# yewsiang/Transferable3D

Measured on AMD Instinct MI355X. Metric: frustums/sec fwd+bwd, higher is better.
Workload: dtype f32

## Files before the change

transferable3d_amd/csrc/bn_optim.hip:

```cpp
#include "common.h"
#include "poolbwd_dev.h"
#include "bn_dev.h"

namespace {

template <int GR, int CH = FC_CH>
__global__ __launch_bounds__(GR * CH) void k_bn_fwd_finalize(const t3d_bn_fwd_finalize_args p) {
  __shared__ double red[GR][CH];
  __shared__ float s_scsh[2 * CH];
  bn_fwd_finalize_body<GR, CH>(p, red, s_scsh, blockIdx.x);
}

__global__ __launch_bounds__(256) void k_pool_finalize(const t3d_pool_finalize_args p) {
  const int i = blockIdx.x * blockDim.x + threadIdx.x;
  if (i >= p.B * p.N) return;
  const int b = i / p.N, c = i % p.N;
  pool_pick_impl(p.pmax, p.pmin, p.pamax, p.pamin, p.tiles_per_frustum, p.N, b, c, p.scale[c], p.shift[c], p.pooled, p.ld_pooled,
                 p.argidx, p.ysel);
}

template <int GR, int CH = FC_CH>
__global__ __launch_bounds__(GR * CH) void k_bn_bwd_finalize(const t3d_bn_bwd_finalize_args p) {
  __shared__ double red[GR][CH];
  bn_bwd_finalize_body<GR, CH>(p, red, blockIdx.x, threadIdx.x);
}

__global__ __launch_bounds__(256) void k_dy_colsum(const t3d_dy_colsum_args p) { dy_colsum_body(p, blockIdx.x, threadIdx.x); }

__global__ __launch_bounds__(256) void k_reduce_slabs(const float* __restrict__ slab_base, float* __restrict__ grad_base,
                                                      const t3d_slab_desc* __restrict__ table) {
  __shared__ float4 part[8][32];
  reduce_slabs_body(slab_base, grad_base, table, part, blockIdx.x, blockIdx.y, gridDim.x);
}

__global__ __launch_bounds__(256) void k_pool_bwd_mid(const float* __restrict__ slab_base, float* __restrict__ grad_base,
                                                      const t3d_slab_desc* __restrict__ table, const int gx, const int n_reduce,
                                                      const t3d_pool_sparse_rows_args sp) {
  extern __shared__ __attribute__((aligned(16))) float smem[];
  const int b = blockIdx.x;
  if (b < n_reduce) {
    reduce_slabs_body(slab_base, grad_base, table, reinterpret_cast<float4(*)[32]>(smem), b % gx, b / gx, gx);
  } else {
    const int r = b - n_reduce, tiles = sp.B * sp.rows_per_frustum / 128;
    pool_sparse_rows_body(sp, smem, r % tiles, r / tiles);
  }
}

__global__ __launch_bounds__(64) void k_schedule_step(float* hyper, const t3d_schedule s) {
  if (blockIdx.x != 0) return;
  schedule_step_body(hyper, s, threadIdx.x);
}

__global__ __launch_bounds__(256) void k_adam_tf(float* __restrict__ w, const float* __restrict__ g, float* __restrict__ m,
                                                 float* __restrict__ v, int64_t n, const float* __restrict__ hyper,
                                                 float b1, float b2, float eps, float gscale) {
  const float lr_t = hyper[3];
  for (int64_t i = (int64_t)blockIdx.x * blockDim.x + threadIdx.x; i < n; i += (int64_t)gridDim.x * blockDim.x) {
    float mi = m[i], vi = v[i];
    const float dw = adam_tf_elem(g[i], mi, vi, lr_t, b1, b2, eps, gscale);
    m[i] = mi;
    v[i] = vi;
    w[i] -= dw;
  }
}

constexpr int ADAM_RANGE_ELEMS = 1024;
__global__ __launch_bounds__(256) void k_reduce_slabs_adam(const float* __restrict__ slab_base, float* __restrict__ grad_base,
                                                           const t3d_slab_desc* __restrict__ table, const int gx, const int n_reduce,
                                                           const t3d_adam_range* __restrict__ ranges, const int n_ranges,
                                                           const adam_tail ad) {
  __shared__ float4 part[8][32];
  const int b = blockIdx.x;
  if (b < n_reduce) {
    reduce_slabs_body<true>(slab_base, grad_base, table, part, b % gx, b / gx, gx, &ad);
    return;
  }
  const int r = b - n_reduce;
  int lo = 0, hi = n_ranges - 1;
  while (lo < hi) {
    const int mid = (lo + hi + 1) >> 1;
    if (ranges[mid].blk0 <= r) lo = mid; else hi = mid - 1;
  }
  const t3d_adam_range rg = ranges[lo];
  const float lr_t = ad.hyper[3];
  const int64_t i0 = (int64_t)(r - rg.blk0) * ADAM_RANGE_ELEMS + threadIdx.x;
#pragma unroll
  for (int u = 0; u < ADAM_RANGE_ELEMS / 256; ++u) {
    const int64_t i = i0 + 256 * u;
    if (i < rg.n) {
      const int64_t o = rg.off + i;
      float mi = ad.m[o], vi = ad.v[o];
      const float dw = adam_tf_elem(grad_base[o], mi, vi, lr_t, ad.b1, ad.b2, ad.eps, ad.gscale);
      ad.m[o] = mi;
      ad.v[o] = vi;
      ad.w[o] -= dw;
    }
  }
}

__global__ __launch_bounds__(256) void k_momentum_tf(float* __restrict__ w, const float* __restrict__ g, float* __restrict__ acc,
                                                     int64_t n, const float* __restrict__ hyper, float momentum, float gscale) {
  const float lr = hyper[1];
  for (int64_t i = (int64_t)blockIdx.x * blockDim.x + threadIdx.x; i < n; i += (int64_t)gridDim.x * blockDim.x) {
    const float a = fmaf(momentum, acc[i], g[i] * gscale);
    acc[i] = a;
    w[i] -= lr * a;
  }
}

__device__ __forceinline__ uint32_t mix_u32(uint64_t x) {
  x ^= x >> 33; x *= 0xff51afd7ed558ccdULL;
  x ^= x >> 33; x *= 0xc4ceb9fe1a85ec53ULL;
  x ^= x >> 33;
  return (uint32_t)(x >> 16);
}
__global__ __launch_bounds__(256) void k_dropout_mask(float* __restrict__ mask, int64_t n, float keep, uint32_t seed,
                                                      const float* __restrict__ hyper) {
  const uint64_t step = (uint64_t)hyper[0];
  const uint64_t key = ((uint64_t)seed << 32) ^ (step * 0x9E3779B97F4A7C15ULL);
  for (int64_t i = (int64_t)blockIdx.x * blockDim.x + threadIdx.x; i < n; i += (int64_t)gridDim.x * blockDim.x) {
    const uint32_t r = mix_u32(key + (uint64_t)i * 0xD6E8FEB86659FD93ULL);
    const float u = (float)(r >> 8) * (1.0f / 16777216.0f);
    mask[i] = u < keep ? 1.f : 0.f;
  }
}

}

extern "C" int t3d_abi_version(void) { return T3D_ABI_VERSION; }

static int fin_big_tiles() {
  static const int v = []() { const char* e = getenv("T3D_FIN_BIG"); const int x = e ? atoi(e) : 512; return x > 0 ? x : (1 << 30); }();
  return v;
}

static int fin_wide_tiles() {
  static const int v = []() { const char* e = getenv("T3D_FIN_WIDE"); const int x = e ? atoi(e) : 1024; return x > 0 ? x : (1 << 30); }();
  return v;
}

extern "C" int t3d_bn_fwd_finalize(const t3d_bn_fwd_finalize_args* a, t3d_stream_t stream) {
  if (!a || !a->gamma || !a->beta || !a->moving_mean || !a->moving_var || !a->scale || !a->shift || !a->mean ||
      !a->invstd)
    return T3D_ERR_ARG;
  if (a->is_training && (!a->psum || !a->psumsq || !a->decay || a->count <= 0)) return T3D_ERR_ARG;
  if (a->is_training && a->n_tiles >= fin_wide_tiles() && a->N <= FC_WIDE_MAX_N)
    T3D_LAUNCH((k_bn_fwd_finalize<FC_GR_WIDE, FC_CH_WIDE>), dim3((a->N + FC_CH_WIDE - 1) / FC_CH_WIDE), dim3(FC_GR_WIDE * FC_CH_WIDE), 0,
               static_cast<hipStream_t>(stream), *a);
  else if (a->is_training && a->n_tiles > fin_big_tiles())
    T3D_LAUNCH(k_bn_fwd_finalize<FC_GR_BIG>, dim3((a->N + FC_CH - 1) / FC_CH), dim3(FC_GR_BIG * FC_CH), 0, static_cast<hipStream_t>(stream), *a);
  else
    T3D_LAUNCH(k_bn_fwd_finalize<FC_GR>, dim3((a->N + FC_CH - 1) / FC_CH), dim3(FC_GR * FC_CH), 0, static_cast<hipStream_t>(stream), *a);
  T3D_CHECK_LAUNCH();
  return T3D_OK;
}

extern "C" int t3d_pool_finalize(const t3d_pool_finalize_args* a, t3d_stream_t stream) {
  if (!a || !a->scale || !a->shift || !a->pmax || !a->pmin || !a->pamax || !a->pamin || !a->pooled || !a->argidx ||
      !a->ysel)
    return T3D_ERR_ARG;
  T3D_LAUNCH(k_pool_finalize, dim3((a->B * a->N + 255) / 256), dim3(256), 0, static_cast<hipStream_t>(stream),
                     *a);
  T3D_CHECK_LAUNCH();
  return T3D_OK;
}

extern "C" int t3d_bn_bwd_finalize(const t3d_bn_bwd_finalize_args* a, t3d_stream_t stream) {
  const int rc = check_bn_bwd_finalize(a);
  if (rc != T3D_OK) return rc;
  if (a->psum_dz != nullptr && a->n_tiles >= fin_wide_tiles() && a->N <= FC_WIDE_MAX_N)
    T3D_LAUNCH((k_bn_bwd_finalize<FC_GR_WIDE, FC_CH_WIDE>), dim3((a->N + FC_CH_WIDE - 1) / FC_CH_WIDE), dim3(FC_GR_WIDE * FC_CH_WIDE), 0,
               static_cast<hipStream_t>(stream), *a);
  else if (a->psum_dz != nullptr && a->n_tiles > fin_big_tiles())
    T3D_LAUNCH(k_bn_bwd_finalize<FC_GR_BIG>, dim3((a->N + FC_CH - 1) / FC_CH), dim3(FC_GR_BIG * FC_CH), 0, static_cast<hipStream_t>(stream), *a);
  else
    T3D_LAUNCH(k_bn_bwd_finalize<FC_GR>, dim3((a->N + FC_CH - 1) / FC_CH), dim3(FC_GR * FC_CH), 0, static_cast<hipStream_t>(stream), *a);
  T3D_CHECK_LAUNCH();
  return T3D_OK;
}

extern "C" int t3d_dy_colsum(const t3d_dy_colsum_args* a, t3d_stream_t stream) {
  const int rc = check_dy_colsum(a);
  if (rc != T3D_OK) return rc;
  T3D_LAUNCH(k_dy_colsum, dim3((a->B * a->N + 255) / 256), dim3(256), 0, static_cast<hipStream_t>(stream), *a);
  T3D_CHECK_LAUNCH();
  return T3D_OK;
}

extern "C" int t3d_reduce_slabs(const float* slab_base, float* grad_base, const t3d_slab_desc* table_dev, int n_tensors,
                                int max_numel, t3d_stream_t stream) {
  if (!slab_base || !grad_base || !table_dev || n_tensors <= 0) return T3D_ERR_ARG;
  int gx = (max_numel / 4 + 31) / 32;
  if (gx > 256) gx = 256;
  if (gx < 1) gx = 1;
  T3D_LAUNCH(k_reduce_slabs, dim3(gx, n_tensors), dim3(256), 0, static_cast<hipStream_t>(stream), slab_base,
                     grad_base, table_dev);
  T3D_CHECK_LAUNCH();
  return T3D_OK;
}

extern "C" int t3d_schedule_step(float* hyper, const t3d_schedule* s, t3d_stream_t stream) {
  if (!hyper || !s) return T3D_ERR_ARG;
  T3D_LAUNCH(k_schedule_step, dim3(1), dim3(64), 0, static_cast<hipStream_t>(stream), hyper, *s);
  T3D_CHECK_LAUNCH();
  return T3D_OK;
}

extern "C" int t3d_adam_tf_step(float* params, const float* grads, float* m, float* v, int64_t n, const float* hyper,
                                float beta1, float beta2, float eps, float grad_scale, t3d_stream_t stream) {
  if (!params || !grads || !m || !v || !hyper || n <= 0) return T3D_ERR_ARG;
  int64_t blocks = (n + 255) / 256;
  if (blocks > 2048) blocks = 2048;
  T3D_LAUNCH(k_adam_tf, dim3((unsigned)blocks), dim3(256), 0, static_cast<hipStream_t>(stream), params, grads, m,
                     v, n, hyper, beta1, beta2, eps, grad_scale);
  T3D_CHECK_LAUNCH();
  return T3D_OK;
}

extern "C" int t3d_reduce_slabs_adam(const float* slab_base, float* grad_base, const t3d_slab_desc* table_dev, int n_tensors,
                                     int max_numel, float* params, float* m, float* v, const t3d_adam_range* ranges_dev, int n_ranges,
                                     int n_range_blocks, const float* hyper, float beta1, float beta2, float eps, float grad_scale,
                                     t3d_stream_t stream) {
  if (!slab_base || !grad_base || !table_dev || n_tensors <= 0 || !params || !m || !v || !hyper) return T3D_ERR_ARG;
  if (n_ranges < 0 || n_range_blocks < 0 || (n_ranges == 0) != (n_range_blocks == 0) || (n_ranges > 0 && !ranges_dev)) return T3D_ERR_ARG;
  int gx = (max_numel / 4 + 31) / 32;
  if (gx > 256) gx = 256;
  if (gx < 1) gx = 1;
  const int n_reduce = gx * n_tensors;
  const adam_tail ad = {params, m, v, hyper, beta1, beta2, eps, grad_scale};
  T3D_LAUNCH(k_reduce_slabs_adam, dim3(n_reduce + n_range_blocks), dim3(256), 0, static_cast<hipStream_t>(stream), slab_base, grad_base,
             table_dev, gx, n_reduce, ranges_dev, n_ranges, ad);
  T3D_CHECK_LAUNCH();
  return T3D_OK;
}

extern "C" int t3d_momentum_step(float* params, const float* grads, float* accum, int64_t n, const float* hyper, float momentum,
                                 float grad_scale, t3d_stream_t stream) {
  if (!params || !grads || !accum || !hyper || n <= 0) return T3D_ERR_ARG;
  int64_t blocks = (n + 255) / 256;
  if (blocks > 2048) blocks = 2048;
  T3D_LAUNCH(k_momentum_tf, dim3((unsigned)blocks), dim3(256), 0, static_cast<hipStream_t>(stream), params, grads, accum, n, hyper,
             momentum, grad_scale);
  T3D_CHECK_LAUNCH();
  return T3D_OK;
}

__global__ __launch_bounds__(256) void k_cast_bf16(const float* __restrict__ src, bf16_t* __restrict__ dst, int64_t n) {
  const int64_t stride = (int64_t)gridDim.x * 256 * 8;
  for (int64_t i = ((int64_t)blockIdx.x * 256 + threadIdx.x) * 8; i < n; i += stride) {
    if (i + 8 <= n) {
      const float4 a = *reinterpret_cast<const float4*>(src + i), b = *reinterpret_cast<const float4*>(src + i + 4);
      const bf16x8 h = {(bf16_t)a.x, (bf16_t)a.y, (bf16_t)a.z, (bf16_t)a.w, (bf16_t)b.x, (bf16_t)b.y, (bf16_t)b.z, (bf16_t)b.w};
      *reinterpret_cast<bf16x8*>(dst + i) = h;
    } else {
      for (int64_t j = i; j < n; ++j) dst[j] = (bf16_t)src[j];
    }
  }
}

extern "C" int t3d_cast_bf16(const float* src, void* dst, int64_t n, t3d_stream_t stream) {
  if (!src || !dst || n <= 0 || (reinterpret_cast<uintptr_t>(src) & 15) || (reinterpret_cast<uintptr_t>(dst) & 15)) return T3D_ERR_ARG;
  int64_t blocks = (n + 2047) / 2048;
  if (blocks > 2048) blocks = 2048;
  T3D_LAUNCH(k_cast_bf16, dim3((unsigned)blocks), dim3(256), 0, static_cast<hipStream_t>(stream), src, static_cast<bf16_t*>(dst), n);
  T3D_CHECK_LAUNCH();
  return T3D_OK;
}

extern "C" int t3d_dropout_mask(float* mask, int64_t n, float keep_prob, uint32_t seed, const float* hyper,
                                t3d_stream_t stream) {
  if (!mask || !hyper || n <= 0) return T3D_ERR_ARG;
  int64_t blocks = (n + 255) / 256;
  if (blocks > 4096) blocks = 4096;
  T3D_LAUNCH(k_dropout_mask, dim3((unsigned)blocks), dim3(256), 0, static_cast<hipStream_t>(stream), mask, n,
                     keep_prob, seed, hyper);
  T3D_CHECK_LAUNCH();
  return T3D_OK;
}

extern "C" int t3d_pool_bwd_mid(const float* slab_base, float* grad_base, const t3d_slab_desc* table_dev, int n_tensors,
                                int max_numel, const t3d_pool_sparse_rows_args* a, t3d_stream_t stream) {
  if (!slab_base || !grad_base || !table_dev || n_tensors <= 0) return T3D_ERR_ARG;
  const int rc = check_sparse_rows(a);
  if (rc != T3D_OK) return rc;
  int gx = (max_numel / 4 + 31) / 32;
  if (gx > 256) gx = 256;
  if (gx < 1) gx = 1;
  const int n_reduce = gx * n_tensors;
  const long M = (long)a->B * a->rows_per_frustum;
  const int n_sparse = (int)(M / 128) * (a->K / SR_KC);
  const size_t lds = sparse_rows_lds(a->N);
  static size_t allowed = 0;
  if (lds > 64 * 1024 && lds > allowed) {
    (void)hipFuncSetAttribute(reinterpret_cast<const void*>(k_pool_bwd_mid), hipFuncAttributeMaxDynamicSharedMemorySize, (int)lds);
    allowed = lds;
  }
  T3D_LAUNCH(k_pool_bwd_mid, dim3(n_reduce + n_sparse), dim3(256), lds, static_cast<hipStream_t>(stream), slab_base, grad_base,
             table_dev, gx, n_reduce, *a);
  T3D_CHECK_LAUNCH();
  return T3D_OK;
}
```

transferable3d_amd/csrc/poolbwd.hip:

```cpp
#include "poolbwd_dev.h"

namespace {

__global__ __launch_bounds__(256) void k_pool_bwd_prep(const t3d_pool_bwd_prep_args p) {
  extern __shared__ __attribute__((aligned(16))) float smem[];
  pool_bwd_prep_body(p, smem, blockIdx.x, blockIdx.y, blockIdx.z);
}
__global__ __launch_bounds__(256) void k_pool_sparse_rows(const t3d_pool_sparse_rows_args p) {
  extern __shared__ __attribute__((aligned(16))) float smem[];
  pool_sparse_rows_body(p, smem, blockIdx.x, blockIdx.y);
}
template <class XT>
__global__ __launch_bounds__(256) void k_act_colsum(const t3d_act_colsum_args p) {
  extern __shared__ __attribute__((aligned(16))) float smem[];
  act_colsum_body<XT>(p, smem, blockIdx.x);
}
template <class XT>
__global__ __launch_bounds__(256) void k_pool_wgrad_finish(const t3d_pool_wgrad_finish_args p) {
  extern __shared__ __attribute__((aligned(16))) float smem[];
  pool_wgrad_finish_body<XT>(p, smem, blockIdx.x, blockIdx.y);
}

}

extern "C" int t3d_pool_bwd_prep(const t3d_pool_bwd_prep_args* a, t3d_stream_t stream) {
  const int rc = check_prep(a);
  if (rc != T3D_OK) return rc;
  T3D_LAUNCH(k_pool_bwd_prep, dim3(a->K / 32, a->K / 32, (a->N + PCH - 1) / PCH), dim3(256), PREP_LDS,
             static_cast<hipStream_t>(stream), *a);
  T3D_CHECK_LAUNCH();
  return T3D_OK;
}

extern "C" int t3d_pool_sparse_rows(const t3d_pool_sparse_rows_args* a, t3d_stream_t stream) {
  const int rc = check_sparse_rows(a);
  if (rc != T3D_OK) return rc;
  const size_t lds = sparse_rows_lds(a->N);
  static size_t allowed = 0;
  if (lds > 64 * 1024 && lds > allowed) {
    (void)hipFuncSetAttribute(reinterpret_cast<const void*>(k_pool_sparse_rows), hipFuncAttributeMaxDynamicSharedMemorySize,
                              (int)lds);
    allowed = lds;
  }
  const long M = (long)a->B * a->rows_per_frustum;
  T3D_LAUNCH(k_pool_sparse_rows, dim3(M / 128, a->K / SR_KC), dim3(256), lds, static_cast<hipStream_t>(stream), *a);
  T3D_CHECK_LAUNCH();
  return T3D_OK;
}

extern "C" int t3d_act_colsum(const t3d_act_colsum_args* a, t3d_stream_t stream) {
  const int rc = check_colsum(a);
  if (rc != T3D_OK) return rc;
  if (a->a.dtype == T3D_BF16) T3D_LAUNCH(k_act_colsum<bf16_t>, dim3(a->M / 128), dim3(256), COLSUM_LDS, static_cast<hipStream_t>(stream), *a);
  else T3D_LAUNCH(k_act_colsum<float>, dim3(a->M / 128), dim3(256), COLSUM_LDS, static_cast<hipStream_t>(stream), *a);
  T3D_CHECK_LAUNCH();
  return T3D_OK;
}

extern "C" int t3d_pool_wgrad_finish(const t3d_pool_wgrad_finish_args* a, t3d_stream_t stream) {
  const int rc = check_finish(a);
  if (rc != T3D_OK) return rc;
  const size_t lds = finish_lds(a->K);
  if (a->a.dtype == T3D_BF16) T3D_LAUNCH(k_pool_wgrad_finish<bf16_t>, dim3(a->K / FK, a->N / FN), dim3(256), lds, static_cast<hipStream_t>(stream), *a);
  else T3D_LAUNCH(k_pool_wgrad_finish<float>, dim3(a->K / FK, a->N / FN), dim3(256), lds, static_cast<hipStream_t>(stream), *a);
  T3D_CHECK_LAUNCH();
  return T3D_OK;
}
```

Baseline: 28140.

## Add per-wave register-accumulating sparse-rows kernel with counting-sort row bucketing

Adds a new sparse-rows backward path in which each wave gathers the argmax hits for its row subset, counting-sorts them by row in LDS, then streams weight rows with batched, software-pipelined float2 loads and accumulates each output row in registers. It replaces the tiled shared-memory accumulation kernel whenever the per-wave LDS fits in 64KB, both standalone and inside the fused pool_bwd_mid launch, where sparse blocks are now ordered before the reduce blocks. The aim is to avoid touching a large LDS tile per block, at the cost of serial per-wave sorting and inline-asm stores. An environment variable can force the old tiled path.

```diff
diff --git a/transferable3d_amd/csrc/bn_optim.hip b/transferable3d_amd/csrc/bn_optim.hip
--- a/transferable3d_amd/csrc/bn_optim.hip
+++ b/transferable3d_amd/csrc/bn_optim.hip
@@ -1,5 +1,6 @@
 #include "common.h"
 #include "poolbwd_dev.h"
+#include "sparse_rows_dev.h"
 #include "bn_dev.h"
 
 namespace {
@@ -43,6 +44,20 @@
   } else {
     const int r = b - n_reduce, tiles = sp.B * sp.rows_per_frustum / 128;
     pool_sparse_rows_body(sp, smem, r % tiles, r / tiles);
+  }
+}
+
+__global__ __launch_bounds__(256) void k_pool_bwd_mid_reg(const float* __restrict__ slab_base, float* __restrict__ grad_base,
+                                                          const t3d_slab_desc* __restrict__ table, const int gx, const int n_sparse,
+                                                          const t3d_pool_sparse_rows_args sp) {
+  extern __shared__ __attribute__((aligned(16))) float smem[];
+  const int b = blockIdx.x;
+  if (b < n_sparse) {
+    const int tiles = sp.B * sp.rows_per_frustum / 128;
+    pool_sparse_rows_reg_body(sp, reinterpret_cast<int*>(smem), b % tiles, b / tiles);
+  } else {
+    const int r = b - n_sparse;
+    reduce_slabs_body(slab_base, grad_base, table, reinterpret_cast<float4(*)[32]>(smem), r % gx, r / gx, gx);
   }
 }
 
@@ -289,6 +304,13 @@
   const int n_reduce = gx * n_tensors;
   const long M = (long)a->B * a->rows_per_frustum;
   const int n_sparse = (int)(M / 128) * (a->K / SR_KC);
+  if (!sparse_rows_take_tile(a->N)) {
+    const size_t rlds = sparse_rows_reg_lds(a->N) > 8 * 32 * sizeof(float4) ? sparse_rows_reg_lds(a->N) : 8 * 32 * sizeof(float4);
+    T3D_LAUNCH(k_pool_bwd_mid_reg, dim3(n_reduce + n_sparse), dim3(256), rlds, static_cast<hipStream_t>(stream), slab_base, grad_base,
+               table_dev, gx, n_sparse, *a);
+    T3D_CHECK_LAUNCH();
+    return T3D_OK;
+  }
   const size_t lds = sparse_rows_lds(a->N);
   static size_t allowed = 0;
   if (lds > 64 * 1024 && lds > allowed) {
diff --git a/transferable3d_amd/csrc/poolbwd.hip b/transferable3d_amd/csrc/poolbwd.hip
--- a/transferable3d_amd/csrc/poolbwd.hip
+++ b/transferable3d_amd/csrc/poolbwd.hip
@@ -1,4 +1,5 @@
 #include "poolbwd_dev.h"
+#include "sparse_rows_dev.h"
 
 namespace {
 
@@ -9,6 +10,10 @@
 __global__ __launch_bounds__(256) void k_pool_sparse_rows(const t3d_pool_sparse_rows_args p) {
   extern __shared__ __attribute__((aligned(16))) float smem[];
   pool_sparse_rows_body(p, smem, blockIdx.x, blockIdx.y);
+}
+__global__ __launch_bounds__(256) void k_pool_sparse_rows_reg(const t3d_pool_sparse_rows_args p) {
+  extern __shared__ __attribute__((aligned(16))) int smem_i[];
+  pool_sparse_rows_reg_body(p, smem_i, blockIdx.x, blockIdx.y);
 }
 template <class XT>
 __global__ __launch_bounds__(256) void k_act_colsum(const t3d_act_colsum_args p) {
@@ -35,6 +40,12 @@
 extern "C" int t3d_pool_sparse_rows(const t3d_pool_sparse_rows_args* a, t3d_stream_t stream) {
   const int rc = check_sparse_rows(a);
   if (rc != T3D_OK) return rc;
+  const long M = (long)a->B * a->rows_per_frustum;
+  if (!sparse_rows_take_tile(a->N)) {
+    T3D_LAUNCH(k_pool_sparse_rows_reg, dim3(M / 128, a->K / SR_KC), dim3(256), sparse_rows_reg_lds(a->N), static_cast<hipStream_t>(stream), *a);
+    T3D_CHECK_LAUNCH();
+    return T3D_OK;
+  }
   const size_t lds = sparse_rows_lds(a->N);
   static size_t allowed = 0;
   if (lds > 64 * 1024 && lds > allowed) {
@@ -42,7 +53,6 @@
                               (int)lds);
     allowed = lds;
   }
-  const long M = (long)a->B * a->rows_per_frustum;
   T3D_LAUNCH(k_pool_sparse_rows, dim3(M / 128, a->K / SR_KC), dim3(256), lds, static_cast<hipStream_t>(stream), *a);
   T3D_CHECK_LAUNCH();
   return T3D_OK;
diff --git a/transferable3d_amd/csrc/sparse_rows_dev.h b/transferable3d_amd/csrc/sparse_rows_dev.h
--- /dev/null
+++ b/transferable3d_amd/csrc/sparse_rows_dev.h
@@ -0,0 +1,227 @@
+#pragma once
+#include <cstdlib>
+#include <cstring>
+#include "poolbwd_dev.h"
+
+namespace {
+
+#ifndef SRR_BATCH_N
+#define SRR_BATCH_N 16
+#endif
+constexpr int SRR_BATCH = SRR_BATCH_N;
+
+#ifdef T3D_TRACE_SPARSE
+#define SRR_CLOCK(slot) srr_clk[slot] = (int)wall_clock64()
+#else
+#define SRR_CLOCK(slot) do {} while (0)
+#endif
+typedef float srr_f2 __attribute__((ext_vector_type(2)));
+constexpr size_t SRR_MAX_LDS = 64 * 1024;
+
+inline size_t sparse_rows_reg_lds(int N) { return (size_t)4 * (2 * (size_t)N + 64) * sizeof(int); }
+
+inline bool sparse_rows_take_tile(int N) {
+  const char* e = getenv("T3D_SPARSE_ROWS");
+  return (e != nullptr && strcmp(e, "tile") == 0) || sparse_rows_reg_lds(N) > SRR_MAX_LDS;
+}
+
+__device__ __forceinline__ void srr_wave_sync() {
+  __builtin_amdgcn_fence(__ATOMIC_RELEASE, "wavefront");
+  __builtin_amdgcn_wave_barrier();
+  __builtin_amdgcn_fence(__ATOMIC_ACQUIRE, "wavefront");
+}
+
+__device__ __forceinline__ unsigned long long srr_peers(int key, bool ok) {
+  unsigned long long m = __ballot(ok);
+#pragma unroll
+  for (int k = 0; k < 5; ++k) {
+    const bool bit = (key >> k) & 1;
+    const unsigned long long bk = __ballot(bit);
+    m &= bit ? bk : ~bk;
+  }
+  return m;
+}
+
+__device__ __forceinline__ void pool_sparse_rows_reg_body(const t3d_pool_sparse_rows_args& p, int* smem, int bx, int by) {
+  const int tid = threadIdx.x, lane = tid & 63, w = tid >> 6;
+  int* raw = smem + (size_t)w * (2 * p.N + 64);
+  int* srt = raw + p.N;
+  int* cur = srt + p.N;
+  const int row0 = bx * 128, kc0 = by * SR_KC;
+  const int b = row0 / p.rows_per_frustum, rin0 = row0 - b * p.rows_per_frustum;
+  const unsigned long long lt = (1ull << lane) - 1ull;
+  const bool gated = p.row_live != nullptr;
+
+#ifdef T3D_TRACE_SPARSE
+  int srr_clk[4];
+#endif
+  SRR_CLOCK(0);
+  cur[lane] = 0;
+  int cnt = 0;
+  for (int nb = 0; nb < p.N; nb += 64 * SR_PRE) {
+    int rr[SR_PRE];
+#pragma unroll
+    for (int q = 0; q < SR_PRE; ++q) {
+      const int n = nb + 64 * q + lane;
+      rr[q] = p.argidx[(size_t)b * p.N + min(n, p.N - 1)];
+    }
+#pragma unroll
+    for (int q = 0; q < SR_PRE; ++q) {
+      if (nb + 64 * q < p.N) {
+        const int n = nb + 64 * q + lane;
+        const int r = rr[q] - rin0;
+        const bool hit = n < p.N && r >= 0 && r < 128 && (r & 3) == w;
+        const unsigned long long m = __ballot(hit);
+        if (hit) raw[cnt + __popcll(m & lt)] = n | (r << 16);
+        cnt += __popcll(m);
+      }
+    }
+  }
+  cnt = __builtin_amdgcn_readfirstlane(cnt);
+  srr_wave_sync();
+  SRR_CLOCK(1);
+
+  for (int c0 = 0; c0 < cnt; c0 += 64) {
+    const bool ok = c0 + lane < cnt;
+    const int rl = raw[min(c0 + lane, cnt - 1)] >> 18;
+    const unsigned long long peers = srr_peers(rl, ok);
+    int base = 0;
+    if (ok) base = cur[rl];
+    srr_wave_sync();
+    if (ok) cur[rl] = base + __popcll(peers);
+    srr_wave_sync();
+  }
+  const int mycnt = lane < 32 ? cur[lane] : 0;
+  int incl = mycnt;
+#pragma unroll
+  for (int d = 1; d < 32; d *= 2) {
+    const int t = __shfl_up(incl, d, 64);
+    if (lane >= d) incl += t;
+  }
+  srr_wave_sync();
+  if (lane < 32) cur[lane] = incl - mycnt;
+  srr_wave_sync();
+  for (int c0 = 0; c0 < cnt; c0 += 64) {
+    const bool ok = c0 + lane < cnt;
+    const int e = raw[min(c0 + lane, cnt - 1)];
+    const int rl = e >> 18;
+    const unsigned long long peers = srr_peers(rl, ok);
+    int base = 0;
+    if (ok) {
+      base = cur[rl];
+      srt[base + __popcll(peers & lt)] = e;
+    }
+    srr_wave_sync();
+    if (ok) cur[rl] = base + __popcll(peers);
+    srr_wave_sync();
+  }
+
+  SRR_CLOCK(2);
+
+  if (cnt > 0) {
+    const int elast = __builtin_amdgcn_readfirstlane(raw[cnt - 1]);
+    const int rlast = (cnt % SR_UNROLL) != 0 ? elast >> 16 : -1;
+    const float2 wlast = *reinterpret_cast<const float2*>(p.wc + (size_t)(elast & 0xffff) * p.K + kc0 + 2 * lane);
+    srr_f2 acc = {0.f, 0.f};
+    int crow = -1;
+    auto flush = [&]() {
+      if (crow == rlast) {
+        acc.x = fmaf(0.f, wlast.x, acc.x);
+        acc.y = fmaf(0.f, wlast.y, acc.y);
+      }
+      float* dst = p.s + (size_t)(row0 + crow) * p.K + kc0 + 2 * lane;
+      asm volatile("global_store_dwordx2 %0, %1, off" : : "v"(dst), "v"(acc) : "memory");
+    };
+    const int k4 = p.K * (int)sizeof(float), lane8 = kc0 * (int)sizeof(float) + 8 * lane;
+    const char* wcb = reinterpret_cast<const char*>(p.wc);
+    struct Chunk { int off, r, g; unsigned long long begins; };
+    auto chunk = [&](int c0, int row_before) {
+      Chunk c;
+      const int e = srt[min(c0 + lane, cnt - 1)];
+      c.off = (e & 0xffff) * k4;
+      c.r = e >> 16;
+      c.g = __float_as_int(p.dpool[(size_t)b * p.N + (e & 0xffff)]);
+      const int before = __shfl_up(c.r, 1, 64);
+      c.begins = __ballot(c.r != (lane == 0 ? row_before : before));
+      return c;
+    };
+    auto issue = [&](const Chunk& c, int j0, float2 (&wv)[SRR_BATCH]) {
+#pragma unroll
+      for (int u = 0; u < SRR_BATCH; ++u) {
+        const unsigned off = (unsigned)__builtin_amdgcn_readlane(c.off, j0 + u) + (unsigned)lane8;
+        wv[u] = *reinterpret_cast<const float2*>(wcb + off);
+      }
+    };
+    auto sum = [&](const Chunk& c, int j0, int left, const float2 (&wv)[SRR_BATCH]) {
+      if (left >= SRR_BATCH) {
+#pragma unroll
+        for (int u = 0; u < SRR_BATCH; ++u) {
+          if (__builtin_expect((c.begins >> (j0 + u)) & 1ull, 0)) {
+            if (crow >= 0) flush();
+            acc.x = 0.f;
+            acc.y = 0.f;
+            crow = __builtin_amdgcn_readlane(c.r, j0 + u);
+          }
+          const float g = __int_as_float(__builtin_amdgcn_readlane(c.g, j0 + u));
+          acc.x = fmaf(g, wv[u].x, acc.x);
+          acc.y = fmaf(g, wv[u].y, acc.y);
+        }
+      } else {
+#pragma unroll
+        for (int u = 0; u < SRR_BATCH; ++u) {
+          if (u < left) {
+            if (__builtin_expect((c.begins >> (j0 + u)) & 1ull, 0)) {
+              if (crow >= 0) flush();
+              acc.x = 0.f;
+              acc.y = 0.f;
+              crow = __builtin_amdgcn_readlane(c.r, j0 + u);
+            }
+            const float g = __int_as_float(__builtin_amdgcn_readlane(c.g, j0 + u));
+            acc.x = fmaf(g, wv[u].x, acc.x);
+            acc.y = fmaf(g, wv[u].y, acc.y);
+          }
+        }
+      }
+    };
+    static_assert(SRR_BATCH == 16, "four batches per 64-entry chunk, written out below");
+    float2 w0[SRR_BATCH], w1[SRR_BATCH], w2[SRR_BATCH], w3[SRR_BATCH];
+    Chunk c = chunk(0, -1);
+    issue(c, 0, w0);
+    if (cnt > 16) issue(c, 16, w1);
+    if (cnt > 32) issue(c, 32, w2);
+    for (int c0 = 0; c0 < cnt; c0 += 64) {
+      const int left = cnt - c0;
+      const Chunk cn = chunk(c0 + 64, __builtin_amdgcn_readlane(c.r, 63));
+      if (left > 48) issue(c, 48, w3);
+      sum(c, 0, left, w0);
+      if (left > 64) issue(cn, 0, w0);
+      if (left > 16) sum(c, 16, left - 16, w1);
+      if (left > 80) issue(cn, 16, w1);
+      if (left > 32) sum(c, 32, left - 32, w2);
+      if (left > 96) issue(cn, 32, w2);
+      if (left > 48) sum(c, 48, left - 48, w3);
+      c = cn;
+    }
+    flush();
+  }
+  SRR_CLOCK(3);
+
+#ifdef T3D_TRACE_SPARSE
+  const int live_rows = __popcll(__ballot(mycnt > 0));
+  if (gated && by == 0 && lane == 0) {
+    for (int q = 0; q < 4; ++q) p.row_live[row0 + 32 * w + q] = srr_clk[q];
+    p.row_live[row0 + 32 * w + 4] = cnt;
+    p.row_live[row0 + 32 * w + 5] = live_rows;
+  }
+#else
+  if (gated && by == 0 && lane < 32) p.row_live[row0 + 4 * lane + w] = mycnt > 0 ? 1 : 0;
+#endif
+  if (!gated) {
+    const unsigned live = (unsigned)__ballot(mycnt > 0);
+    for (int j = 0; j < 32; ++j)
+      if (!((live >> j) & 1u))
+        *reinterpret_cast<float2*>(p.s + (size_t)(row0 + 4 * j + w) * p.K + kc0 + 2 * lane) = make_float2(0.f, 0.f);
+  }
+}
+
+}
```

After: 28370, median of 6. Within noise of the previous version (+0.8%).
